# nomadkaraoke/python-audio-separator

Hardware: AMD Instinct MI355X
Metric: audio-sec separated / wall-sec (RTF), UVR-MDX-NET 44.1kHz stereo, 1/2/4/8 GPU (higher is better)
Workload: dtype f32 (I/O and accumulators; matrix products on the 16-bit pipe from block-scaled two-part fp16 operands, 22-bit products -- see arithmetic; fp32-exact setting timed in arithmetic_ab)

## Files before the change

python-audio-separator_amd/csrc/asx.hip:

```cpp
#include <hip/hip_runtime.h>

#include <algorithm>
#include <atomic>
#include <cmath>
#include <cstdarg>
#include <cstdio>
#include <cstdlib>
#include <cstring>
#include <functional>
#include <map>
#include <string>
#include <mutex>
#include <vector>

#include "../../include/asx.h"
#include "knobs.h"

static void grant_lds(const void *kernel, int bytes) {
  static std::mutex mu;
  static std::map<const void *, int> granted;
  std::lock_guard<std::mutex> lock(mu);
  int &g = granted[kernel];
  if (bytes > g) {
    (void)hipFuncSetAttribute(kernel, hipFuncAttributeMaxDynamicSharedMemorySize, bytes);
// ... 38 lines not shown
  const char *refusal = nullptr;
  int shipped = 0;
} kOptions[] = {
    {"winograd", &asx_engine::winograd, &EngineKnobs::winograd, opt_nonneg,
     "asx_set_option: winograd = %d names a superseded kernel generation that only an experimental build carries "
     "(python build.py --experimental); this library has 0 (direct kernel) and 3 (the default)", 3},
    {"winograd_stationary", &asx_engine::winos, &EngineKnobs::winos, opt_nonneg,
     "asx_set_option: the weight-stationary Winograd kernel (measured slower) is in experimental builds only (python build.py --experimental)"},
    {"winograd_bf16x6", &asx_engine::wino6, &EngineKnobs::wino6, opt_nonneg},
    {"gemm_bf16x6", &asx_engine::gemm_bf16x6, &EngineKnobs::gemm_bf16x6, opt_onoff},
    {"gemm_f16x3", &asx_engine::gemm_f16x3, &EngineKnobs::gemm_f16x3, opt_onoff},
    {"conv_direct_f16x3", &asx_engine::conv3h, &EngineKnobs::conv3h, opt_nonneg},
    {"conv_fuse_input", &asx_engine::conv_fuse_input, &EngineKnobs::conv_fuse_input, opt_onoff},
    {"conv_down_bf16x6", &asx_engine::down6, &EngineKnobs::down6, opt_onoff},
    {"conv_up_bf16x6", &asx_engine::up6, &EngineKnobs::up6, opt_onoff},
    {"gemm_pair_images", &asx_engine::pair_images, &EngineKnobs::pair_images, opt_onoff,
     "asx_set_option: gemm_pair_images = 1 needs an experimental build (python build.py --experimental): the pair-image reader measured no "
     "faster in the nets and is not in the default library"},
};

static const EngineOption *find_option(const char *fn, const char *key) {
  for (const EngineOption &o : kOptions)
    if (!strcmp(key, o.key)) return &o;
  set_err("%s: unknown option '%s'", fn, key);
  return nullptr;
}

extern "C" {

int asx_abi_version(void) { return ASX_ABI_VERSION; }
// ... 128 lines not shown
static void vr_destroy(VrNet *n);
static void ens_destroy(EnsCtx *c);
static void free_conv(ConvLayer &L) {
  L.w.release();
  L.b.release();
  L.wu.release();
  L.wu2.release();
  L.wu3.release();
  L.wus.release();
  L.wu6.release();
  L.wu6h.release();
  L.w3h.release();
  L.w1f.release();
  L.wd6.release();
  L.wup6.release();
  L.gn_w.release();
  L.gn_b.release();
}
static void free_tdf(TdfLayer &L) {
  L.w.release();
  L.bias.release();
  L.scale.release();
  L.shift.release();
  L.gn_w.release();
  L.gn_b.release();
}
static void free_block(Block &b) {
  for (auto &c : b.tfc) free_conv(c);
  free_tdf(b.tdf0);
  free_tdf(b.tdf1);
// ... 912 lines not shown
    kind = CK_DOWN;
    to = t / 2;
    fo = f / 2;
  } else if (!strcmp(op, "conv1x1")) kind = CK_1X1;
  else if (!strcmp(op, "up")) {
    kind = CK_UP;
    to = 2 * t;
    fo = 2 * f;
    REQUIRE(aux_host, "asx_op_conv(up): skip tensor required");
  } else {
    set_err("asx_op_conv: unknown op '%s'", op);
    return ASX_ERR_INVALID;
  }
  ConvLayer L;
  DevBuf dx, dy, dskip;
  BufGuard g{{&dx, &dy, &dskip, &L.w, &L.b, &L.wu, &L.wu2, &L.wu3, &L.wus, &L.wu6, &L.wu6h, &L.w3h, &L.wd6, &L.wup6}};
  CHK(conv_setup(L, kind, cin, cout, relu ? 1 : 0));
  CHK(conv_pack(L, w_host, b_host, e->winograd));
  CHK(to_dev(dx, x_host, (size_t)B * cin * t * f));
  const size_t ny = (size_t)B * cout * to * fo;
  CHK(dy.ensure(ny * 4));
  HIPCHK(hipMemset(dy.p, 0xff, ny * 4));
  if (kind == CK_UP) CHK(to_dev(dskip, aux_host, ny));
  CHK(conv_launch(e, L, dx.f(), dskip.f(), dy.f(), B, t, f, nullptr));
  CHK(to_host(y_host, dy, ny));
  return ASX_OK;
}

int asx_op_tdf(asx_engine *e, const float *x_host, int32_t B, int32_t c, int32_t t, int32_t k, const float *w_host,
               const float *bias_host, int32_t n, const float *scale_host, const float *shift_host,
               const float *res_host, float *y_host) {
// ... 934 lines not shown
int asx_counter(const asx_engine *e, const char *name, int64_t *out) {
  REQUIRE(e && name && out, "asx_counter: null argument");
  const std::string nm(name);
  if (nm == "tdf3_launches") *out = (int64_t)g_tdf3_launches.load();
  else if (nm == "tdf3h_launches") *out = (int64_t)g_tdf3h_launches.load();
  else if (nm == "attn6_launches") *out = (int64_t)g_attn6_launches.load();
  else if (nm == "attn6h_launches") *out = (int64_t)g_attn6h_launches.load();
  else if (nm == "tdf3_gather_launches") *out = (int64_t)g_tdf3_gather_launches.load();
  else if (nm == "wino6_launches") *out = (int64_t)g_wino6_launches.load();
  else if (nm == "wino6h_launches") *out = (int64_t)g_wino6h_launches.load();
  else if (nm == "conv3h_launches") *out = (int64_t)g_conv3h_launches.load();
  else if (nm == "conv3h_fin_launches") *out = (int64_t)g_conv3h_fin_launches.load();
  else if (nm == "tdf3_pair_image_launches") *out = (int64_t)g_tdf3ps_launches.load();
  else if (nm == "down6_launches") *out = (int64_t)g_down6_launches.load();
  else if (nm == "up6_launches") *out = (int64_t)g_up6_launches.load();
  else if (nm == "hd_rounds") *out = (int64_t)g_hd_rounds.load();
  else {
    set_err("asx_counter: unknown counter '%s'", name);
    return ASX_ERR_INVALID;
  }
  return ASX_OK;
}

int asx_debug_trace(uint64_t *host, int64_t n_u64) {
  REQUIRE(host && n_u64 > 0 && n_u64 <= 4096 * 8, "asx_debug_trace: bad argument");
  HIPCHK(hipDeviceSynchronize());
  HIPCHK(hipMemcpyFromSymbol(host, HIP_SYMBOL(asx_dbg_trace), (size_t)n_u64 * 8));
  return ASX_OK;
}

// ... 199 lines not shown
```

python-audio-separator_amd/csrc/engine_core.h:

```cpp
#pragma once

static thread_local char g_err[512] = "";
static void set_err(const char *fmt, ...) {
  va_list ap;
  va_start(ap, fmt);
  vsnprintf(g_err, sizeof(g_err), fmt, ap);
  va_end(ap);
}
#define HIPCHK(x)                                                                       \
  do {                                                                                  \
    hipError_t e_ = (x);                                                                \
    if (e_ != hipSuccess) {                                                             \
      set_err("%s:%d %s -> %s", __FILE__, __LINE__, #x, hipGetErrorString(e_));         \
      return ASX_ERR_HIP;                                                               \
    }                                                                                   \
  } while (0)
#define CHK(x)                    \
  do {                            \
    int r_ = (x);                 \
    if (r_ != ASX_OK) return r_;  \
  } while (0)
#define REQUIRE(cond, ...)        \
  do {                            \
    if (!(cond)) {                \
// ... 68 lines not shown
  DevBuf wu2;
  DevBuf wu3;
  int wu_cg = 0, wu_nci = 0, wu3_nci = 0;
  DevBuf wus;
  int wus_ks = 0;
  DevBuf gn_w, gn_b;
  DevBuf wu6;
  int wu6_nci = 0;
  DevBuf wu6h;
  DevBuf w3h;
  DevBuf w1f;
  DevBuf wd6;
  int wd6_cg = 0, wd6_nst = 0, wd6_nrep = 3;
  DevBuf wup6;
  int wup6_cg = 0, wup6_nst = 0;
};

struct TdfLayer {
  int n = 0, k = 0, c = 0;
  bool has_bias = false;
  DevBuf w, bias, scale, shift;
  DevBuf gn_w, gn_b;
};

struct Block {
  std::vector<ConvLayer> tfc;
  TdfLayer tdf0, tdf1;
  int c = 0, t = 0, f = 0;
};

// ... 64 lines not shown
  DevBuf d_div;
  DivKey div_key;
  DevBuf sinc_tab;
  hipEvent_t div_ev = nullptr;
  hipStream_t div_stream = nullptr;
  std::vector<DevBuf> skip;
  int winograd = 3;
  int winos = 0;
  int gemm_bf16x6 = 1;
  int gemm_f16x3 = 1;
  int wino6 = 144;
  int conv3h = 144;
  int conv_fuse_input = 1;
  int down6 = 1;
  int up6 = 1;
  int pair_images = 0;
  std::vector<W3Entry> w3;
  std::mutex w3_mu;
  bool prof = false;
  int prof_nprod = 0;
  std::vector<ProfRec> recs;
};

static int pick_batch(const asx_engine *e) { return e->cfg.max_batch > 0 ? e->cfg.max_batch : 64; }

static int even_batches(int nk, int maxB) {
  const int nbatch = (nk + maxB - 1) / maxB;
  return (nk + nbatch - 1) / nbatch;
}

// ... 74 lines not shown
```

python-audio-separator_amd/csrc/engine_mdx.h:

```cpp
#pragma once

template <class CFG>
static void launch_conv_t(const ConvArgs &a, int nblk, hipStream_t s) {
  grant_lds(&conv_mfma_kernel<CFG>, CFG::LDS_BYTES);
  hipLaunchKernelGGL(conv_mfma_kernel<CFG>, dim3(nblk), dim3(256), CFG::LDS_BYTES, s, a);
}

static int conv_tile_h(int kind) { return kind == CK_UP ? 4 : 8; }

static int pick_nrep_conv(int cout) {
  const int ct = (cout + 15) / 16;
  int best = 1, best_pad = 1 << 30;
  for (int n = 3; n >= 1; --n) {
    const int pad = ((ct + n - 1) / n) * n - ct;
    if (pad < best_pad) {
      best_pad = pad;
      best = n;
    }
  }
  return best;
}
static int pick_nrep_up(int cout) {
  const int ct = (cout + 15) / 16;
  if (knobs().up_nrep == 4 && (4 * ct) % 4 == 0) return 4;
// ... 150 lines not shown
  }
  if (L.kind == CK_1X1 && L.cin == 4 && L.cout == Conv3hCfg::C) {
    std::vector<float> w1((size_t)Conv3hCfg::C * 5, 0.f);
    memcpy(w1.data(), w, (size_t)Conv3hCfg::C * 4 * 4);
    if (b) memcpy(w1.data() + Conv3hCfg::C * 4, b, (size_t)Conv3hCfg::C * 4);
    CHK(L.w1f.ensure(w1.size() * 4));
    HIPCHK(hipMemcpy(L.w1f.p, w1.data(), w1.size() * 4, hipMemcpyHostToDevice));
  }
  if (L.kind == CK_DOWN) {
    std::vector<uint32_t> w6;
    L.wd6_nrep = (knobs().down6_wide && L.cout % 96 == 0) ? 6 : 3;
    if (L.wd6_nrep == 6) down6_pack<6>(w, L.cout, L.cin, w6, &L.wd6_cg, &L.wd6_nst);
    else down6_pack<3>(w, L.cout, L.cin, w6, &L.wd6_cg, &L.wd6_nst);
    CHK(L.wd6.ensure(w6.size() * 4));
    HIPCHK(hipMemcpy(L.wd6.p, w6.data(), w6.size() * 4, hipMemcpyHostToDevice));
  }
  if (L.kind == CK_UP) {
    std::vector<uint32_t> w6;
    if (L.nrep == 6) up6_pack<6>(w, L.cout, L.cin, w6, &L.wup6_cg, &L.wup6_nst);
    else if (L.nrep == 4) up6_pack<4>(w, L.cout, L.cin, w6, &L.wup6_cg, &L.wup6_nst);
    else up6_pack<2>(w, L.cout, L.cin, w6, &L.wup6_cg, &L.wup6_nst);
    CHK(L.wup6.ensure(w6.size() * 4));
    HIPCHK(hipMemcpy(L.wup6.p, w6.data(), w6.size() * 4, hipMemcpyHostToDevice));
  }
  const int nb = (L.kind == CK_UP) ? CT * 16 : std::max(L.cg * NW, ((L.cout + 47) / 48) * 48);
  std::vector<float> bp(nb, 0.f);
  for (int i = 0; i < L.cout; ++i) bp[i] = b ? b[i] : 0.f;
  CHK(L.w.ensure(wp.size() * 4));
  CHK(L.b.ensure(bp.size() * 4));
  HIPCHK(hipMemcpy(L.w.p, wp.data(), wp.size() * 4, hipMemcpyHostToDevice));
  HIPCHK(hipMemcpy(L.b.p, bp.data(), bp.size() * 4, hipMemcpyHostToDevice));
  return ASX_OK;
}

template <class CFG>
static void launch_conv_dma_t(const ConvArgs &a, int nblk, hipStream_t s) {
  grant_lds(&conv_dma_kernel<CFG>, CFG::LDS_BYTES);
  hipLaunchKernelGGL(conv_dma_kernel<CFG>, dim3(nblk), dim3(256), CFG::LDS_BYTES, s, a);
}

static std::atomic<long long> g_wino6_launches{0};
static std::atomic<long long> g_wino6h_launches{0};
static std::atomic<long long> g_conv3h_launches{0};
static std::atomic<long long> g_conv3h_fin_launches{0};
static std::atomic<long long> g_down6_launches{0};
static std::atomic<long long> g_up6_launches{0};

struct ConvView {
  int64_t x_bstride = 0;
  int64_t y_bstride = 0;
  const float *res = nullptr;
  int64_t aux_bstride = 0;
  int act = -1;
  float alpha = 1.f;
  const ConvLayer *fin = nullptr;
  const float *fin_x = nullptr;
};

static bool conv3h_takes(const asx_engine *e, const ConvLayer &L, bool dma, const float *res, int act, int T, int F, int64_t y_bstride, const float *y) {
#ifdef ASX_EXPERIMENTAL_KERNELS
  if (e->winos == 1 && L.wus.p != nullptr) return false;
// ... 227 lines not shown
    wa.wp = L.wu.f();
    wa.CG = L.wu_cg;
    wa.NCI = L.wu_nci;
    wa.tilesT = (a.To + WinoCfg::TH - 1) / WinoCfg::TH;
    wa.tilesF = (a.Fo + WinoCfg::TW - 1) / WinoCfg::TW;
    const int nb = wa.CG * wa.tilesT * wa.tilesF * B;
    grant_lds(&conv_wino_kernel, WinoCfg::LDS_BYTES);
    return timed(e, cls, flops, bytes, s, [&]() {
      hipLaunchKernelGGL(conv_wino_kernel, dim3(nb), dim3(256), WinoCfg::LDS_BYTES, s, wa);
    });
  }
#endif
  if (L.kind == CK_DOWN && e->gemm_bf16x6 > 0 && e->down6 > 0 && L.wd6.p != nullptr && dma && (a.Fo & 3) == 0 && (reinterpret_cast<uintptr_t>(y) & 15) == 0 &&
      a.y_bstride % 4 == 0 && (v.res == nullptr || ((reinterpret_cast<uintptr_t>(v.res) & 15) == 0 && a.aux_bstride % 4 == 0))) {
    ConvArgs da = a;
    da.wp = reinterpret_cast<const float *>(L.wd6.p);
    da.CG = L.wd6_cg;
    da.NCI = L.wd6_nst;
    da.tilesT = (a.To + Down6Cfg::TH - 1) / Down6Cfg::TH;
    da.tilesF = (a.Fo + Down6Cfg::TW - 1) / Down6Cfg::TW;
    const int nb6 = da.CG * da.tilesT * da.tilesF * B;
    grant_lds(&conv_down6_kernel<3>, Down6CfgT<3>::LDS_BYTES);
    grant_lds(&conv_down6_kernel<6>, Down6CfgT<6>::LDS_BYTES);
    g_down6_launches.fetch_add(1);
    return timed(e, cls, flops, bytes, s, [&]() {
      e->prof_nprod = 6;
      if (L.wd6_nrep == 6) hipLaunchKernelGGL(conv_down6_kernel<6>, dim3(nb6), dim3(256), Down6CfgT<6>::LDS_BYTES, s, da);
      else hipLaunchKernelGGL(conv_down6_kernel<3>, dim3(nb6), dim3(256), Down6CfgT<3>::LDS_BYTES, s, da);
    });
  }
  if (L.kind == CK_UP && e->gemm_bf16x6 > 0 && e->up6 > 0 && L.wup6.p != nullptr && dma && (reinterpret_cast<uintptr_t>(y) & 15) == 0 && a.y_bstride % 4 == 0 &&
      (skip == nullptr || ((reinterpret_cast<uintptr_t>(skip) & 15) == 0 && a.aux_bstride % 4 == 0))) {
    ConvArgs ua = a;
    ua.wp = reinterpret_cast<const float *>(L.wup6.p);
    ua.CG = L.wup6_cg;
    ua.NCI = L.wup6_nst;
    ua.tilesT = (T + 1) / 2;
    ua.tilesF = (F + 63) / 64;
    const int nbu = ua.CG * ua.tilesT * ua.tilesF * B;
    grant_lds(&conv_up6_kernel<6>, Up6CfgT<6>::LDS_BYTES);
    grant_lds(&conv_up6_kernel<4>, Up6CfgT<4>::LDS_BYTES);
    grant_lds(&conv_up6_kernel<2>, Up6CfgT<2>::LDS_BYTES);
    g_up6_launches.fetch_add(1);
    return timed(e, cls, flops, bytes, s, [&]() {
      e->prof_nprod = 6;
      if (L.nrep == 6) hipLaunchKernelGGL(conv_up6_kernel<6>, dim3(nbu), dim3(256), Up6CfgT<6>::LDS_BYTES, s, ua);
      else if (L.nrep == 4) hipLaunchKernelGGL(conv_up6_kernel<4>, dim3(nbu), dim3(256), Up6CfgT<4>::LDS_BYTES, s, ua);
      else hipLaunchKernelGGL(conv_up6_kernel<2>, dim3(nbu), dim3(256), Up6CfgT<2>::LDS_BYTES, s, ua);
    });
  }
#define ASX_CONV_CASE(KH, KW, S, PAD, NR, KC, RPW, EPI)                                      \
  do {                                                                                       \
    if (dma) launch_conv_dma_t<ConvDmaCfg<KH, KW, S, PAD, NR, KC, RPW, EPI>>(d, nblk, s);    \
    else launch_conv_t<ConvCfg<KH, KW, S, PAD, NR, KC, RPW, EPI>>(a, nblk, s);               \
  } while (0)
  CHK(timed(e, cls, flops, bytes, s, [&]() {
    switch (L.kind) {
      case CK_3X3:
        if (L.nrep == 3 && L.kc == 4) ASX_CONV_CASE(3, 3, 1, 1, 3, 4, 2, EPI_BIAS_ACT);
        else if (L.nrep == 3) ASX_CONV_CASE(3, 3, 1, 1, 3, 8, 2, EPI_BIAS_ACT);
        else if (L.nrep == 2 && L.kc == 4) ASX_CONV_CASE(3, 3, 1, 1, 2, 4, 2, EPI_BIAS_ACT);
// ... 690 lines not shown
```

python-audio-separator_amd/csrc/kernels_updown6.h:

```cpp
#pragma once
#include "kernels_gemm3.h"

namespace asx {

template <int NREP_, int TH_ = 2>
struct Down6CfgT {
  static constexpr int TH = TH_, TW = 64, KC = 8, NREP = NREP_, NW = 16 * NREP_;
  static constexpr int IH = 2 * TH, IWA = 2 * TW;
  static constexpr int PLANE = IH * IWA;
  static constexpr int NJ = PLANE / 256;
  static constexpr int PAIRS = TH / 2;
  static constexpr int PS = PLANE + 16;
  static constexpr int XBYTES = KC * PS * 4;
  static constexpr int WSTAGE_U32 = 3 * NREP * 64 * 4;
  static constexpr int BUF = XBYTES + WSTAGE_U32 * 4;
  static constexpr int LDS_BYTES = BUF;
};
typedef Down6CfgT<3> Down6Cfg;

static inline uint16_t down6_bf16_rne(float v) {
  uint32_t u;
  memcpy(&u, &v, 4);
  if ((u & 0x7f800000u) == 0x7f800000u) return (uint16_t)((u >> 16) | ((u & 0xffffu) ? 0x40u : 0u));
  u += 0x7fffu + ((u >> 16) & 1u);
  return (uint16_t)(u >> 16);
}
static inline float down6_bf16_f(uint16_t h) {
  const uint32_t u = (uint32_t)h << 16;
  float f;
  memcpy(&f, &u, 4);
  return f;
}

template <int NREP>
static inline void down6_pack(const float *w, int cout, int cin, std::vector<uint32_t> &img, int *cg_out, int *nst_out) {
  using Down6Cfg = Down6CfgT<NREP>;
  const int cg = (cout + Down6Cfg::NW - 1) / Down6Cfg::NW, nst = (cin + Down6Cfg::KC - 1) / Down6Cfg::KC;
  img.assign((size_t)cg * nst * Down6Cfg::WSTAGE_U32, 0u);
  uint16_t *o = reinterpret_cast<uint16_t *>(img.data());
  for (int g = 0; g < cg; ++g)
    for (int st = 0; st < nst; ++st)
      for (int n = 0; n < Down6Cfg::NREP; ++n)
        for (int lane = 0; lane < 64; ++lane) {
          const int co = g * Down6Cfg::NW + n * 16 + (lane & 15), lk = lane >> 4;
          for (int e = 0; e < 2; ++e)
            for (int tap = 0; tap < 4; ++tap) {
              const int c = st * Down6Cfg::KC + 2 * lk + e;
              const float v = (co < cout && c < cin) ? w[((size_t)co * cin + c) * 4 + tap] : 0.f;
              const uint16_t h = down6_bf16_rne(v);
              const float r1 = v - down6_bf16_f(h);
              const uint16_t m = down6_bf16_rne(r1);
              const uint16_t l = down6_bf16_rne(r1 - down6_bf16_f(m));
              const uint16_t parts[3] = {h, m, l};
              for (int p = 0; p < 3; ++p)
                o[((((size_t)(g * nst + st) * 3 + p) * Down6Cfg::NREP + n) * 64 + lane) * 8 + e * 4 + tap] = parts[p];
            }
        }
  if (cg_out) *cg_out = cg;
  if (nst_out) *nst_out = nst;
}

template <int NREP>
__device__ __forceinline__ void updown6_products(const u32x4 *w_s, int lane, const bf16x8 (&xh)[2], const bf16x8 (&xm)[2], const bf16x8 (&xl)[2],
// ... 15 lines not shown
    for (int n = 0; n < NREP; ++n) acc[m][n] = ASX_MFMA_BF16(xh[m], bw[n], acc[m][n]);
  }
#pragma unroll
  for (int n = 0; n < NREP; ++n) bw[n] = __builtin_bit_cast(bf16x8, w_s[n * 64 + lane]);
#pragma unroll
  for (int m = 0; m < 2; ++m) {
#pragma unroll
    for (int n = 0; n < NREP; ++n) acc[m][n] = ASX_MFMA_BF16(xl[m], bw[n], acc[m][n]);
#pragma unroll
    for (int n = 0; n < NREP; ++n) acc[m][n] = ASX_MFMA_BF16(xm[m], bw[n], acc[m][n]);
#pragma unroll
    for (int n = 0; n < NREP; ++n) acc[m][n] = ASX_MFMA_BF16(xh[m], bw[n], acc[m][n]);
  }
}

template <int NREP, int TH = 2>
__global__ __launch_bounds__(256, TH == 2 ? 4 : 3) void conv_down6_kernel(ConvArgs a) {
  using C = Down6CfgT<NREP, TH>;
  extern __shared__ float lds_f[];
  char *lds = reinterpret_cast<char *>(lds_f);
  const int tid = threadIdx.x, lane = tid & 63;
  const int wave = __builtin_amdgcn_readfirstlane(tid >> 6);
  const int li = lane & 15, lk = lane >> 4;

  int lid = xcd_remap(blockIdx.x, gridDim.x);
  const int cg = lid % a.CG;
  lid /= a.CG;
  const int tf = lid % a.tilesF;
  lid /= a.tilesF;
  const int tt = lid % a.tilesT;
  const int b = lid / a.tilesT;
  const int to0 = tt * C::TH, fo0 = tf * C::TW;
  const int ti0 = 2 * to0, fa0 = 2 * fo0;
// ... 17 lines not shown
    uint32_t *w_s = reinterpret_cast<uint32_t *>(lds + buf * C::BUF + C::XBYTES);
#pragma unroll
    for (int p = 0; p < 2; ++p) {
      const int pl = wave + 4 * p;
      const int c = st * C::KC + pl;
      const float *xc = xb + (int64_t)c * plane_sz;
      const bool cok = c < a.Cin;
#pragma unroll
      for (int j = 0; j < C::NJ; ++j) {
        const float *src = (cok && sp_ok[j]) ? xc + sp_off[j] : a.zeros;
        ASX_GLDS16(src, in_s + pl * C::PS + j * 256);
      }
    }
    const uint32_t *ws = wg + (int64_t)st * C::WSTAGE_U32;
#pragma unroll
    for (int i = 0; i < (3 * C::NREP + 3) / 4; ++i) {
      const int q = wave + 4 * i;
      if (q < 3 * C::NREP) ASX_GLDS16(ws + q * 256 + lane * 4, w_s + q * 256);
    }
  };

  f32x4 acc[C::PAIRS][2][C::NREP];
#pragma unroll
  for (int pi = 0; pi < C::PAIRS; ++pi)
#pragma unroll
    for (int m = 0; m < 2; ++m)
#pragma unroll
      for (int n = 0; n < C::NREP; ++n) acc[pi][m][n] = (f32x4){0.f, 0.f, 0.f, 0.f};

  const int row = TH == 2 ? (wave >> 1) : wave;
  for (int st = 0; st < a.NCI; ++st) {
    if (st > 0) __syncthreads();
    issue(st, 0);
    asm volatile("s_waitcnt vmcnt(0)" ::: "memory");
    __syncthreads();
    const float *in_s = reinterpret_cast<const float *>(lds);
    const u32x4 *w_s = reinterpret_cast<const u32x4 *>(lds + C::XBYTES);
#pragma unroll
    for (int pi = 0; pi < C::PAIRS; ++pi) {
      const int col0 = TH == 2 ? (wave & 1) * 2 : 2 * pi;
      bf16x8 xh[2], xm[2], xl[2];
#pragma unroll
      for (int m = 0; m < 2; ++m) {
        const float *p0 = in_s + (2 * lk) * C::PS + (2 * row) * C::IWA + 2 * ((col0 + m) * 16 + li);
        const f32x2 c0d0 = *reinterpret_cast<const f32x2 *>(p0);
        const f32x2 c0d1 = *reinterpret_cast<const f32x2 *>(p0 + C::IWA);
        const f32x2 c1d0 = *reinterpret_cast<const f32x2 *>(p0 + C::PS);
        const f32x2 c1d1 = *reinterpret_cast<const f32x2 *>(p0 + C::PS + C::IWA);
        unsigned hh[4], mm[4], ll[4];
        split3_pair(c0d0.x, c0d0.y, hh[0], mm[0], ll[0]);
        split3_pair(c0d1.x, c0d1.y, hh[1], mm[1], ll[1]);
        split3_pair(c1d0.x, c1d0.y, hh[2], mm[2], ll[2]);
        split3_pair(c1d1.x, c1d1.y, hh[3], mm[3], ll[3]);
        xh[m] = __builtin_bit_cast(bf16x8, (u32x4){hh[0], hh[1], hh[2], hh[3]});
        xm[m] = __builtin_bit_cast(bf16x8, (u32x4){mm[0], mm[1], mm[2], mm[3]});
        xl[m] = __builtin_bit_cast(bf16x8, (u32x4){ll[0], ll[1], ll[2], ll[3]});
      }
      updown6_products<C::NREP>(w_s, lane, xh, xm, xl, acc[pi]);
    }
  }

  const int t = to0 + row;
  if (t >= a.To) return;
  float *yb = a.y + (int64_t)b * a.y_bstride;
  const float *rb = a.res ? a.res + (int64_t)b * a.aux_bstride : nullptr;
#pragma unroll
  for (int n = 0; n < C::NREP; ++n) {
    const int co = cg * C::NW + n * 16 + li;
    if (co >= a.Cout) continue;
    const float bv = a.bias[co];
#pragma unroll
    for (int pi = 0; pi < C::PAIRS; ++pi)
#pragma unroll
      for (int m = 0; m < 2; ++m) {
        const int col0 = TH == 2 ? (wave & 1) * 2 : 2 * pi;
        const int f = fo0 + (col0 + m) * 16 + lk * 4;
        const int64_t off = ((int64_t)co * a.To + t) * a.Fo + f;
        const f32x4 v = acc[pi][m][n];
        if ((a.Fo & 3) == 0 && f + 4 <= a.Fo) {
          f32x4 o;
          o.x = act_fn(v.x + bv, a.act);
          o.y = act_fn(v.y + bv, a.act);
          o.z = act_fn(v.z + bv, a.act);
          o.w = act_fn(v.w + bv, a.act);
          if (rb != nullptr) o += *reinterpret_cast<const f32x4 *>(rb + off);
          *reinterpret_cast<f32x4 *>(yb + off) = o;
        } else {
          const float ov[4] = {v.x, v.y, v.z, v.w};
#pragma unroll
          for (int r = 0; r < 4; ++r)
            if (f + r < a.Fo) yb[off + r] = act_fn(ov[r] + bv, a.act) + (rb != nullptr ? rb[off + r] : 0.f);
        }
      }
  }
}

template <int NREP_>
struct Up6CfgT {
  static constexpr int TH = 2, TW = 64, KC = 32, NREP = NREP_;
  static constexpr int PAIR = 2 * TH * TW + 16;
  static constexpr int XBYTES = (KC / 2) * PAIR * 4;
  static constexpr int WSTAGE_U32 = 3 * NREP * 64 * 4;
  static constexpr int BUF = XBYTES + WSTAGE_U32 * 4;
  static constexpr int NBUF = 1;
  static constexpr int LDS_BYTES = NBUF * BUF;
};

template <int NREP>
static inline void up6_pack(const float *w, int cout, int cin, std::vector<uint32_t> &img, int *cg_out, int *nst_out) {
  using C = Up6CfgT<NREP>;
  const int CT = (cout + 15) / 16, vt = 4 * CT;
  const int cg = (vt + NREP - 1) / NREP, nst = (cin + C::KC - 1) / C::KC;
  img.assign((size_t)cg * nst * C::WSTAGE_U32, 0u);
  uint16_t *o = reinterpret_cast<uint16_t *>(img.data());
  for (int g = 0; g < cg; ++g)
    for (int st = 0; st < nst; ++st)
      for (int n = 0; n < NREP; ++n) {
        const int nt = g * NREP + n, pair = nt / 2, dx = nt & 1, dy = pair / CT, ct = pair % CT;
        for (int lane = 0; lane < 64; ++lane) {
          const int co = ct * 16 + (lane & 15), lk = lane >> 4;
          for (int kk = 0; kk < 8; ++kk) {
            const int c = st * C::KC + 2 * (lk + 4 * (kk >> 1)) + (kk & 1);
            const float v = (dy < 2 && co < cout && c < cin) ? w[(((size_t)c * cout + co) * 2 + dy) * 2 + dx] : 0.f;
            const uint16_t h = down6_bf16_rne(v);
            const float r1 = v - down6_bf16_f(h);
            const uint16_t m = down6_bf16_rne(r1);
            const uint16_t l = down6_bf16_rne(r1 - down6_bf16_f(m));
            const uint16_t parts[3] = {h, m, l};
            for (int p = 0; p < 3; ++p) o[((((size_t)(g * nst + st) * 3 + p) * NREP + n) * 64 + lane) * 8 + kk] = parts[p];
          }
        }
      }
  if (cg_out) *cg_out = cg;
  if (nst_out) *nst_out = nst;
}

template <int NREP>
__global__ __launch_bounds__(256, 4) void conv_up6_kernel(ConvArgs a) {
  using C = Up6CfgT<NREP>;
  static_assert(NREP % 2 == 0, "the dx tiles of a pair stay together");
  extern __shared__ float lds_f[];
  char *lds = reinterpret_cast<char *>(lds_f);
  const int tid = threadIdx.x, lane = tid & 63;
  const int wave = __builtin_amdgcn_readfirstlane(tid >> 6);
  const int li = lane & 15, lk = lane >> 4;

  int lid = xcd_remap(blockIdx.x, gridDim.x);
  const int cg = lid % a.CG;
  lid /= a.CG;
  const int tf = lid % a.tilesF;
  lid /= a.tilesF;
  const int tt = lid % a.tilesT;
  const int b = lid / a.tilesT;
  const int to0 = tt * C::TH, fo0 = tf * C::TW;
// ... 5 lines not shown
  const int slot = lane & 31, srow = slot >> 4, sc4 = slot & 15;
  const bool sp_ok = (to0 + srow) < a.T && (fo0 + sc4 * 4) < a.F;
  const int sp_off = (to0 + srow) * a.F + fo0 + sc4 * 4;
  auto issue = [&](int st, int buf) {
    float *in_s = reinterpret_cast<float *>(lds + buf * C::BUF);
    uint32_t *w_s = reinterpret_cast<uint32_t *>(lds + buf * C::BUF + C::XBYTES);
#pragma unroll
    for (int i = 0; i < 4; ++i) {
      const int pr = wave + 4 * i;
      const int c = st * C::KC + 2 * pr + (lane >> 5);
      const float *src = (c < a.Cin && sp_ok) ? xb + (int64_t)c * plane_sz + sp_off : a.zeros;
      ASX_GLDS16(src, in_s + pr * C::PAIR);
    }
    const uint32_t *ws = wg + (int64_t)st * C::WSTAGE_U32;
#pragma unroll
    for (int i = 0; i < (3 * NREP + 3) / 4; ++i) {
      const int q = wave + 4 * i;
      if (q < 3 * NREP) ASX_GLDS16(ws + q * 256 + lane * 4, w_s + q * 256);
    }
  };

  f32x4 acc[2][NREP];
#pragma unroll
  for (int m = 0; m < 2; ++m)
#pragma unroll
    for (int n = 0; n < NREP; ++n) acc[m][n] = (f32x4){0.f, 0.f, 0.f, 0.f};

  const int row = wave >> 1, col0 = (wave & 1) * 2;
  for (int st = 0; st < a.NCI; ++st) {
    if (st > 0) __syncthreads();
    issue(st, 0);
    asm volatile("s_waitcnt vmcnt(0)" ::: "memory");
    __syncthreads();
    const float *in_s = reinterpret_cast<const float *>(lds);
    const u32x4 *w_s = reinterpret_cast<const u32x4 *>(lds + C::XBYTES);
    bf16x8 xh[2], xm[2], xl[2];
#pragma unroll
    for (int m = 0; m < 2; ++m) {
      const float *p0 = in_s + lk * C::PAIR + row * C::TW + (col0 + m) * 16 + li;
      unsigned hh[4], mm[4], ll[4];
#pragma unroll
      for (int jj = 0; jj < 4; ++jj) {
        const float v0 = p0[jj * 4 * C::PAIR], v1 = p0[jj * 4 * C::PAIR + C::TH * C::TW];
        split3_pair(v0, v1, hh[jj], mm[jj], ll[jj]);
      }
      xh[m] = __builtin_bit_cast(bf16x8, (u32x4){hh[0], hh[1], hh[2], hh[3]});
      xm[m] = __builtin_bit_cast(bf16x8, (u32x4){mm[0], mm[1], mm[2], mm[3]});
      xl[m] = __builtin_bit_cast(bf16x8, (u32x4){ll[0], ll[1], ll[2], ll[3]});
    }
    updown6_products<NREP>(w_s, lane, xh, xm, xl, acc);
// ... 1 lines not shown

  const int t = to0 + row;
  if (t >= a.T) return;
  const int CT = (a.Cout + 15) / 16;
  const int To2 = a.T * 2, Fo2 = a.F * 2;
  float *yb = a.y + (int64_t)b * a.y_bstride;
  const float *sb = a.skip ? a.skip + (int64_t)b * a.aux_bstride : nullptr;
#pragma unroll
  for (int np = 0; np < NREP / 2; ++np) {
    const int pair = (cg * NREP) / 2 + np;
    const int dy = pair / CT, ct = pair - dy * CT;
    if (dy >= 2) continue;
    const int co = ct * 16 + li;
    if (co >= a.Cout) continue;
    const float bv = a.bias[co];
    f32x4 s0[2], s1[2];
#pragma unroll
    for (int m = 0; m < 2; ++m) {
      const int f = fo0 + (col0 + m) * 16 + lk * 4;
      const int64_t off = ((int64_t)co * To2 + (2 * t + dy)) * Fo2 + 2 * f;
      const bool in = sb != nullptr && f + 4 <= a.F;
      s0[m] = in ? *reinterpret_cast<const f32x4 *>(sb + off) : (f32x4){1.f, 1.f, 1.f, 1.f};
      s1[m] = in ? *reinterpret_cast<const f32x4 *>(sb + off + 4) : (f32x4){1.f, 1.f, 1.f, 1.f};
    }
#pragma unroll
    for (int m = 0; m < 2; ++m) {
      const int f = fo0 + (col0 + m) * 16 + lk * 4;
      if (f >= a.F) continue;
      const int64_t off = ((int64_t)co * To2 + (2 * t + dy)) * Fo2 + 2 * f;
      const f32x4 v0 = acc[m][2 * np], v1 = acc[m][2 * np + 1];
      if (f + 4 <= a.F) {
        f32x4 r0, r1;
        r0.x = act_fn(v0.x + bv, a.act);
        r0.y = act_fn(v1.x + bv, a.act);
        r0.z = act_fn(v0.y + bv, a.act);
        r0.w = act_fn(v1.y + bv, a.act);
        r1.x = act_fn(v0.z + bv, a.act);
        r1.y = act_fn(v1.z + bv, a.act);
        r1.z = act_fn(v0.w + bv, a.act);
        r1.w = act_fn(v1.w + bv, a.act);
        r0 *= s0[m];
        r1 *= s1[m];
        *reinterpret_cast<f32x4 *>(yb + off) = r0;
        *reinterpret_cast<f32x4 *>(yb + off + 4) = r1;
      } else {
// ... 11 lines not shown
```

python-audio-separator_amd/csrc/knobs.h:

```cpp
#pragma once

#include <algorithm>
#include <climits>
#include <cstdint>
#include <cstdlib>

#ifndef ASX_TDF2_DEFAULT
#define ASX_TDF2_DEFAULT 1
#endif

constexpr int HD_MAX_GROUPS = 6;

namespace knob {
inline bool set(const char *name) { return getenv(name) != nullptr; }
inline int num(const char *name, int def) { return set(name) ? atoi(getenv(name)) : def; }
inline int64_t num64(const char *name, int64_t def) { return set(name) ? atoll(getenv(name)) : def; }
inline double real(const char *name, double def) { return set(name) ? atof(getenv(name)) : def; }
inline bool on_unless_0(const char *name) { return !(set(name) && atoi(getenv(name)) == 0); }
inline bool off_unless_nonzero(const char *name) { return set(name) && atoi(getenv(name)) != 0; }
inline int clamped(const char *name, int def, int lo, int hi = INT_MAX) { return set(name) ? std::max(lo, std::min(hi, atoi(getenv(name)))) : def; }
}

struct Knobs {
  int poison = knob::num("ASX_POISON", -1);
// ... 68 lines not shown
  int winograd = knob::clamped("ASX_WINOGRAD", 3, 0);
  int winos = knob::clamped("ASX_WINOS", 0, 0);
  int pair_images = knob::num("ASX_PAIR_IMAGES", 0);
#else
  int winograd = knob::num("ASX_WINOGRAD", 3) <= 0 ? 0 : 3;
  int winos = 0;
  int pair_images = 0;
#endif
  int gemm_bf16x6 = knob::num("ASX_GEMM_BF16X6", 1);
  int gemm_f16x3 = knob::num("ASX_GEMM_F16X3", 1);
  int wino6 = knob::clamped("ASX_WINO6", 144, 0);
  int conv3h = knob::clamped("ASX_CONV3H", 144, 0);
  int conv_fuse_input = 1;
  int down6 = knob::num("ASX_DOWN6", 1);
  int up6 = knob::num("ASX_UP6", 1);
  bool fft3 = knob::on_unless_0("ASX_FFT3");
  bool fft3p = knob::on_unless_0("ASX_FFT3P");
};
```

Before: 1578.

## Add block-scaled two-part fp16 variants of the down/up convolution kernels

Adds f16x3 variants of the strided down-conv and transposed up-conv kernels. Weights are packed as scaled fp16 hi/lo pairs with a per-output-channel exponent, and activations are split on the fly with a running wave-wide exponent. This needs three MFMA products per tile instead of six bf16 products, and the weight tile staged in LDS shrinks from three parts to two. The variants are on by default whenever gemm_f16x3 is enabled. The cost is more in-kernel work for the activation split and rescaling, plus a different rounding profile that depends on the dynamic exponent tracking.

```diff
diff --git a/python-audio-separator_amd/csrc/asx.hip b/python-audio-separator_amd/csrc/asx.hip
--- a/python-audio-separator_amd/csrc/asx.hip
+++ b/python-audio-separator_amd/csrc/asx.hip
@@ -76,6 +76,7 @@
     {"conv_fuse_input", &asx_engine::conv_fuse_input, &EngineKnobs::conv_fuse_input, opt_onoff},
     {"conv_down_bf16x6", &asx_engine::down6, &EngineKnobs::down6, opt_onoff},
     {"conv_up_bf16x6", &asx_engine::up6, &EngineKnobs::up6, opt_onoff},
+    {"conv_updown_f16x3", &asx_engine::updown_f16x3, &EngineKnobs::updown_f16x3, opt_onoff},
     {"gemm_pair_images", &asx_engine::pair_images, &EngineKnobs::pair_images, opt_onoff,
      "asx_set_option: gemm_pair_images = 1 needs an experimental build (python build.py --experimental): the pair-image reader measured no "
      "faster in the nets and is not in the default library"},
@@ -234,6 +235,8 @@
   L.w1f.release();
   L.wd6.release();
   L.wup6.release();
+  L.wd6h.release();
+  L.wup6h.release();
   L.gn_w.release();
   L.gn_b.release();
 }
@@ -1176,7 +1179,7 @@
   }
   ConvLayer L;
   DevBuf dx, dy, dskip;
-  BufGuard g{{&dx, &dy, &dskip, &L.w, &L.b, &L.wu, &L.wu2, &L.wu3, &L.wus, &L.wu6, &L.wu6h, &L.w3h, &L.wd6, &L.wup6}};
+  BufGuard g{{&dx, &dy, &dskip, &L.w, &L.b, &L.wu, &L.wu2, &L.wu3, &L.wus, &L.wu6, &L.wu6h, &L.w3h, &L.wd6, &L.wup6, &L.wd6h, &L.wup6h}};
   CHK(conv_setup(L, kind, cin, cout, relu ? 1 : 0));
   CHK(conv_pack(L, w_host, b_host, e->winograd));
   CHK(to_dev(dx, x_host, (size_t)B * cin * t * f));
@@ -2141,6 +2144,8 @@
   else if (nm == "tdf3_pair_image_launches") *out = (int64_t)g_tdf3ps_launches.load();
   else if (nm == "down6_launches") *out = (int64_t)g_down6_launches.load();
   else if (nm == "up6_launches") *out = (int64_t)g_up6_launches.load();
+  else if (nm == "down6h_launches") *out = (int64_t)g_down6h_launches.load();
+  else if (nm == "up6h_launches") *out = (int64_t)g_up6h_launches.load();
   else if (nm == "hd_rounds") *out = (int64_t)g_hd_rounds.load();
   else {
     set_err("asx_counter: unknown counter '%s'", name);
diff --git a/python-audio-separator_amd/csrc/engine_core.h b/python-audio-separator_amd/csrc/engine_core.h
--- a/python-audio-separator_amd/csrc/engine_core.h
+++ b/python-audio-separator_amd/csrc/engine_core.h
@@ -106,6 +106,7 @@
   int wd6_cg = 0, wd6_nst = 0, wd6_nrep = 3;
   DevBuf wup6;
   int wup6_cg = 0, wup6_nst = 0;
+  DevBuf wd6h, wup6h;
 };
 
 struct TdfLayer {
@@ -200,6 +201,7 @@
   int conv_fuse_input = 1;
   int down6 = 1;
   int up6 = 1;
+  int updown_f16x3 = 1;
   int pair_images = 0;
   std::vector<W3Entry> w3;
   std::mutex w3_mu;
diff --git a/python-audio-separator_amd/csrc/engine_mdx.h b/python-audio-separator_amd/csrc/engine_mdx.h
--- a/python-audio-separator_amd/csrc/engine_mdx.h
+++ b/python-audio-separator_amd/csrc/engine_mdx.h
@@ -188,6 +188,10 @@
     else down6_pack<3>(w, L.cout, L.cin, w6, &L.wd6_cg, &L.wd6_nst);
     CHK(L.wd6.ensure(w6.size() * 4));
     HIPCHK(hipMemcpy(L.wd6.p, w6.data(), w6.size() * 4, hipMemcpyHostToDevice));
+    if (L.wd6_nrep == 6) down6_pack<6, true>(w, L.cout, L.cin, w6, nullptr, nullptr);
+    else down6_pack<3, true>(w, L.cout, L.cin, w6, nullptr, nullptr);
+    CHK(L.wd6h.ensure(w6.size() * 4));
+    HIPCHK(hipMemcpy(L.wd6h.p, w6.data(), w6.size() * 4, hipMemcpyHostToDevice));
   }
   if (L.kind == CK_UP) {
     std::vector<uint32_t> w6;
@@ -196,6 +200,11 @@
     else up6_pack<2>(w, L.cout, L.cin, w6, &L.wup6_cg, &L.wup6_nst);
     CHK(L.wup6.ensure(w6.size() * 4));
     HIPCHK(hipMemcpy(L.wup6.p, w6.data(), w6.size() * 4, hipMemcpyHostToDevice));
+    if (L.nrep == 6) up6_pack<6, true>(w, L.cout, L.cin, w6, nullptr, nullptr);
+    else if (L.nrep == 4) up6_pack<4, true>(w, L.cout, L.cin, w6, nullptr, nullptr);
+    else up6_pack<2, true>(w, L.cout, L.cin, w6, nullptr, nullptr);
+    CHK(L.wup6h.ensure(w6.size() * 4));
+    HIPCHK(hipMemcpy(L.wup6h.p, w6.data(), w6.size() * 4, hipMemcpyHostToDevice));
   }
   const int nb = (L.kind == CK_UP) ? CT * 16 : std::max(L.cg * NW, ((L.cout + 47) / 48) * 48);
   std::vector<float> bp(nb, 0.f);
@@ -219,6 +228,9 @@
 static std::atomic<long long> g_conv3h_fin_launches{0};
 static std::atomic<long long> g_down6_launches{0};
 static std::atomic<long long> g_up6_launches{0};
+static std::atomic<long long> g_down6h_launches{0};
+static std::atomic<long long> g_up6h_launches{0};
+constexpr int UPDOWN_H_MIN_CIN = 0;
 
 struct ConvView {
   int64_t x_bstride = 0;
@@ -476,7 +488,8 @@
   if (L.kind == CK_DOWN && e->gemm_bf16x6 > 0 && e->down6 > 0 && L.wd6.p != nullptr && dma && (a.Fo & 3) == 0 && (reinterpret_cast<uintptr_t>(y) & 15) == 0 &&
       a.y_bstride % 4 == 0 && (v.res == nullptr || ((reinterpret_cast<uintptr_t>(v.res) & 15) == 0 && a.aux_bstride % 4 == 0))) {
     ConvArgs da = a;
-    da.wp = reinterpret_cast<const float *>(L.wd6.p);
+    const bool h3 = e->gemm_f16x3 > 0 && e->updown_f16x3 > 0 && L.wd6h.p != nullptr && L.cin >= UPDOWN_H_MIN_CIN;
+    da.wp = reinterpret_cast<const float *>(h3 ? L.wd6h.p : L.wd6.p);
     da.CG = L.wd6_cg;
     da.NCI = L.wd6_nst;
     da.tilesT = (a.To + Down6Cfg::TH - 1) / Down6Cfg::TH;
@@ -484,17 +497,23 @@
     const int nb6 = da.CG * da.tilesT * da.tilesF * B;
     grant_lds(&conv_down6_kernel<3>, Down6CfgT<3>::LDS_BYTES);
     grant_lds(&conv_down6_kernel<6>, Down6CfgT<6>::LDS_BYTES);
+    grant_lds(&conv_down6_kernel<3, 2, true>, Down6CfgT<3, 2, true>::LDS_BYTES);
+    grant_lds(&conv_down6_kernel<6, 2, true>, Down6CfgT<6, 2, true>::LDS_BYTES);
     g_down6_launches.fetch_add(1);
+    if (h3) g_down6h_launches.fetch_add(1);
     return timed(e, cls, flops, bytes, s, [&]() {
-      e->prof_nprod = 6;
-      if (L.wd6_nrep == 6) hipLaunchKernelGGL(conv_down6_kernel<6>, dim3(nb6), dim3(256), Down6CfgT<6>::LDS_BYTES, s, da);
+      e->prof_nprod = h3 ? 3 : 6;
+      if (h3 && L.wd6_nrep == 6) hipLaunchKernelGGL((conv_down6_kernel<6, 2, true>), dim3(nb6), dim3(256), (Down6CfgT<6, 2, true>::LDS_BYTES), s, da);
+      else if (h3) hipLaunchKernelGGL((conv_down6_kernel<3, 2, true>), dim3(nb6), dim3(256), (Down6CfgT<3, 2, true>::LDS_BYTES), s, da);
+      else if (L.wd6_nrep == 6) hipLaunchKernelGGL(conv_down6_kernel<6>, dim3(nb6), dim3(256), Down6CfgT<6>::LDS_BYTES, s, da);
       else hipLaunchKernelGGL(conv_down6_kernel<3>, dim3(nb6), dim3(256), Down6CfgT<3>::LDS_BYTES, s, da);
     });
   }
   if (L.kind == CK_UP && e->gemm_bf16x6 > 0 && e->up6 > 0 && L.wup6.p != nullptr && dma && (reinterpret_cast<uintptr_t>(y) & 15) == 0 && a.y_bstride % 4 == 0 &&
       (skip == nullptr || ((reinterpret_cast<uintptr_t>(skip) & 15) == 0 && a.aux_bstride % 4 == 0))) {
     ConvArgs ua = a;
-    ua.wp = reinterpret_cast<const float *>(L.wup6.p);
+    const bool h3 = e->gemm_f16x3 > 0 && e->updown_f16x3 > 0 && L.wup6h.p != nullptr && L.cin >= UPDOWN_H_MIN_CIN;
+    ua.wp = reinterpret_cast<const float *>(h3 ? L.wup6h.p : L.wup6.p);
     ua.CG = L.wup6_cg;
     ua.NCI = L.wup6_nst;
     ua.tilesT = (T + 1) / 2;
@@ -503,10 +522,17 @@
     grant_lds(&conv_up6_kernel<6>, Up6CfgT<6>::LDS_BYTES);
     grant_lds(&conv_up6_kernel<4>, Up6CfgT<4>::LDS_BYTES);
     grant_lds(&conv_up6_kernel<2>, Up6CfgT<2>::LDS_BYTES);
+    grant_lds(&conv_up6_kernel<6, true>, Up6CfgHT<6, true>::LDS_BYTES);
+    grant_lds(&conv_up6_kernel<4, true>, Up6CfgHT<4, true>::LDS_BYTES);
+    grant_lds(&conv_up6_kernel<2, true>, Up6CfgHT<2, true>::LDS_BYTES);
     g_up6_launches.fetch_add(1);
+    if (h3) g_up6h_launches.fetch_add(1);
     return timed(e, cls, flops, bytes, s, [&]() {
-      e->prof_nprod = 6;
-      if (L.nrep == 6) hipLaunchKernelGGL(conv_up6_kernel<6>, dim3(nbu), dim3(256), Up6CfgT<6>::LDS_BYTES, s, ua);
+      e->prof_nprod = h3 ? 3 : 6;
+      if (h3 && L.nrep == 6) hipLaunchKernelGGL((conv_up6_kernel<6, true>), dim3(nbu), dim3(256), (Up6CfgHT<6, true>::LDS_BYTES), s, ua);
+      else if (h3 && L.nrep == 4) hipLaunchKernelGGL((conv_up6_kernel<4, true>), dim3(nbu), dim3(256), (Up6CfgHT<4, true>::LDS_BYTES), s, ua);
+      else if (h3) hipLaunchKernelGGL((conv_up6_kernel<2, true>), dim3(nbu), dim3(256), (Up6CfgHT<2, true>::LDS_BYTES), s, ua);
+      else if (L.nrep == 6) hipLaunchKernelGGL(conv_up6_kernel<6>, dim3(nbu), dim3(256), Up6CfgT<6>::LDS_BYTES, s, ua);
       else if (L.nrep == 4) hipLaunchKernelGGL(conv_up6_kernel<4>, dim3(nbu), dim3(256), Up6CfgT<4>::LDS_BYTES, s, ua);
       else hipLaunchKernelGGL(conv_up6_kernel<2>, dim3(nbu), dim3(256), Up6CfgT<2>::LDS_BYTES, s, ua);
     });
diff --git a/python-audio-separator_amd/csrc/kernels_updown6.h b/python-audio-separator_amd/csrc/kernels_updown6.h
--- a/python-audio-separator_amd/csrc/kernels_updown6.h
+++ b/python-audio-separator_amd/csrc/kernels_updown6.h
@@ -1,10 +1,12 @@
 #pragma once
 #include "kernels_gemm3.h"
+#include "kernels_conv3h.h"
 
 namespace asx {
 
-template <int NREP_, int TH_ = 2>
+template <int NREP_, int TH_ = 2, bool H_ = false>
 struct Down6CfgT {
+  static constexpr int WPARTS = H_ ? 2 : 3;
   static constexpr int TH = TH_, TW = 64, KC = 8, NREP = NREP_, NW = 16 * NREP_;
   static constexpr int IH = 2 * TH, IWA = 2 * TW;
   static constexpr int PLANE = IH * IWA;
@@ -12,7 +14,7 @@
   static constexpr int PAIRS = TH / 2;
   static constexpr int PS = PLANE + 16;
   static constexpr int XBYTES = KC * PS * 4;
-  static constexpr int WSTAGE_U32 = 3 * NREP * 64 * 4;
+  static constexpr int WSTAGE_U32 = WPARTS * NREP * 64 * 4;
   static constexpr int BUF = XBYTES + WSTAGE_U32 * 4;
   static constexpr int LDS_BYTES = BUF;
 };
@@ -32,12 +34,53 @@
   return f;
 }
 
-template <int NREP>
+static inline uint16_t down6_f16_rne(float v) {
+  uint32_t u;
+  memcpy(&u, &v, 4);
+  const uint16_t sign = (uint16_t)((u >> 16) & 0x8000u);
+  const float a = std::fabs(v);
+  if (!(a == a)) return (uint16_t)(sign | 0x7e00u);
+  if (a < 6.103515625e-5f) return (uint16_t)(sign | (uint16_t)std::nearbyint(std::ldexp((double)a, 24)));
+  if (a >= 65520.f) return (uint16_t)(sign | 0x7c00u);
+  int e;
+  const double f = std::frexp((double)a, &e);
+  int m = (int)std::nearbyint(std::ldexp(f, 11));
+  if (m == 2048) {
+    m = 1024;
+    ++e;
+  }
+  return (uint16_t)(sign | ((e - 1 + 15) << 10) | (m - 1024));
+}
+static inline float down6_f16_f(uint16_t h) {
+  const int ex = (h >> 10) & 31, m = h & 0x3ff;
+  float f;
+  if (ex == 0) f = std::ldexp((float)m, -24);
+  else if (ex == 31) f = m ? NAN : INFINITY;
+  else f = std::ldexp((float)(1024 + m), ex - 25);
+  return (h & 0x8000u) ? -f : f;
+}
+static inline int down6_f16_exp(float mx) {
+  if (!(mx > 0.f) || std::isinf(mx)) return 0;
+  int fe;
+  (void)std::frexp(mx, &fe);
+  return 15 - fe;
+}
+
+template <int NREP, bool H = false>
 static inline void down6_pack(const float *w, int cout, int cin, std::vector<uint32_t> &img, int *cg_out, int *nst_out) {
-  using Down6Cfg = Down6CfgT<NREP>;
+  using Down6Cfg = Down6CfgT<NREP, 2, H>;
   const int cg = (cout + Down6Cfg::NW - 1) / Down6Cfg::NW, nst = (cin + Down6Cfg::KC - 1) / Down6Cfg::KC;
-  img.assign((size_t)cg * nst * Down6Cfg::WSTAGE_U32, 0u);
+  img.assign((size_t)cg * nst * Down6Cfg::WSTAGE_U32 + (H ? (size_t)cg * Down6Cfg::NW : 0), 0u);
   uint16_t *o = reinterpret_cast<uint16_t *>(img.data());
+  std::vector<int> ex(H ? (size_t)cg * Down6Cfg::NW : 0, 0);
+  if (H) {
+    for (int co = 0; co < cout; ++co) {
+      float mx = 0.f;
+      for (int i = 0; i < cin * 4; ++i) mx = std::max(mx, std::fabs(w[(size_t)co * cin * 4 + i]));
+      ex[co] = down6_f16_exp(mx);
+      img[(size_t)cg * nst * Down6Cfg::WSTAGE_U32 + co] = (uint32_t)ex[co];
+    }
+  }
   for (int g = 0; g < cg; ++g)
     for (int st = 0; st < nst; ++st)
       for (int n = 0; n < Down6Cfg::NREP; ++n)
@@ -47,6 +90,13 @@
             for (int tap = 0; tap < 4; ++tap) {
               const int c = st * Down6Cfg::KC + 2 * lk + e;
               const float v = (co < cout && c < cin) ? w[((size_t)co * cin + c) * 4 + tap] : 0.f;
+              if (H) {
+                const float vs = std::ldexp(v, ex[co]);
+                const uint16_t hh = down6_f16_rne(vs), lh = down6_f16_rne(vs - down6_f16_f(hh));
+                o[((((size_t)(g * nst + st) * 2 + 0) * Down6Cfg::NREP + n) * 64 + lane) * 8 + e * 4 + tap] = hh;
+                o[((((size_t)(g * nst + st) * 2 + 1) * Down6Cfg::NREP + n) * 64 + lane) * 8 + e * 4 + tap] = lh;
+                continue;
+              }
               const uint16_t h = down6_bf16_rne(v);
               const float r1 = v - down6_bf16_f(h);
               const uint16_t m = down6_bf16_rne(r1);
@@ -92,9 +142,52 @@
   }
 }
 
-template <int NREP, int TH = 2>
+template <int NREP>
+__device__ __forceinline__ void updown6_products(const u32x4 *w_s, int lane, const f16x8 (&xh)[2], const f16x8 (&xl)[2], f32x4 (&acc)[2][NREP]) {
+  f16x8 bw[NREP];
+#pragma unroll
+  for (int n = 0; n < NREP; ++n) bw[n] = __builtin_bit_cast(f16x8, w_s[(NREP + n) * 64 + lane]);
+#pragma unroll
+  for (int m = 0; m < 2; ++m)
+#pragma unroll
+    for (int n = 0; n < NREP; ++n) acc[m][n] = ASX_MFMA_F16(xh[m], bw[n], acc[m][n]);
+#pragma unroll
+  for (int n = 0; n < NREP; ++n) bw[n] = __builtin_bit_cast(f16x8, w_s[n * 64 + lane]);
+#pragma unroll
+  for (int m = 0; m < 2; ++m) {
+#pragma unroll
+    for (int n = 0; n < NREP; ++n) acc[m][n] = ASX_MFMA_F16(xl[m], bw[n], acc[m][n]);
+#pragma unroll
+    for (int n = 0; n < NREP; ++n) acc[m][n] = ASX_MFMA_F16(xh[m], bw[n], acc[m][n]);
+  }
+}
+
+template <int NREP>
+__device__ __forceinline__ void updown6_split_h(const float (&v)[8], int &em, int &em_lo, f32x4 (&acc)[NREP], f16x8 &xh, f16x8 &xl) {
+  float mx = fmaxf(fmaxf(fmaxf(fabsf(v[0]), fabsf(v[1])), fmaxf(fabsf(v[2]), fabsf(v[3]))), fmaxf(fmaxf(fabsf(v[4]), fabsf(v[5])), fmaxf(fabsf(v[6]), fabsf(v[7]))));
+  mx = wave_max64(mx);
+  const int need = min(__builtin_amdgcn_readfirstlane(f16_scale_exp(mx)), 100);
+  int e_new = em;
+  if (need < em) e_new = need - 2;
+  else if (need > em + F16X3_RISE && mx > 0.f) e_new = min(need - 2, em_lo + F16X3_RISE_CAP);
+  em_lo = min(em_lo, e_new);
+  if (e_new != em) {
+    const float fdev = __builtin_ldexpf(1.0f, e_new - em);
+#pragma unroll
+    for (int n = 0; n < NREP; ++n) acc[n] *= fdev;
+  }
+  em = e_new;
+  const float sc = __builtin_ldexpf(1.0f, e_new);
+  unsigned hh[4], ll[4];
+#pragma unroll
+  for (int i = 0; i < 4; ++i) conv3h_split_pair(v[2 * i], v[2 * i + 1], sc, hh[i], ll[i]);
+  xh = __builtin_bit_cast(f16x8, (u32x4){hh[0], hh[1], hh[2], hh[3]});
+  xl = __builtin_bit_cast(f16x8, (u32x4){ll[0], ll[1], ll[2], ll[3]});
+}
+
+template <int NREP, int TH = 2, bool H = false>
 __global__ __launch_bounds__(256, TH == 2 ? 4 : 3) void conv_down6_kernel(ConvArgs a) {
-  using C = Down6CfgT<NREP, TH>;
+  using C = Down6CfgT<NREP, TH, H>;
   extern __shared__ float lds_f[];
   char *lds = reinterpret_cast<char *>(lds_f);
   const int tid = threadIdx.x, lane = tid & 63;
@@ -142,12 +235,17 @@
     }
     const uint32_t *ws = wg + (int64_t)st * C::WSTAGE_U32;
 #pragma unroll
-    for (int i = 0; i < (3 * C::NREP + 3) / 4; ++i) {
+    for (int i = 0; i < (C::WPARTS * C::NREP + 3) / 4; ++i) {
       const int q = wave + 4 * i;
-      if (q < 3 * C::NREP) ASX_GLDS16(ws + q * 256 + lane * 4, w_s + q * 256);
+      if (q < C::WPARTS * C::NREP) ASX_GLDS16(ws + q * 256 + lane * 4, w_s + q * 256);
     }
   };
 
+  int em[C::PAIRS][2], em_lo[C::PAIRS][2];
+#pragma unroll
+  for (int pi = 0; pi < C::PAIRS; ++pi)
+#pragma unroll
+    for (int m = 0; m < 2; ++m) em[pi][m] = em_lo[pi][m] = 200;
   f32x4 acc[C::PAIRS][2][C::NREP];
 #pragma unroll
   for (int pi = 0; pi < C::PAIRS; ++pi)
@@ -167,6 +265,21 @@
 #pragma unroll
     for (int pi = 0; pi < C::PAIRS; ++pi) {
       const int col0 = TH == 2 ? (wave & 1) * 2 : 2 * pi;
+      if constexpr (H) {
+        f16x8 fh[2], fl[2];
+#pragma unroll
+        for (int m = 0; m < 2; ++m) {
+          const float *p0 = in_s + (2 * lk) * C::PS + (2 * row) * C::IWA + 2 * ((col0 + m) * 16 + li);
+          const f32x2 c0d0 = *reinterpret_cast<const f32x2 *>(p0);
+          const f32x2 c0d1 = *reinterpret_cast<const f32x2 *>(p0 + C::IWA);
+          const f32x2 c1d0 = *reinterpret_cast<const f32x2 *>(p0 + C::PS);
+          const f32x2 c1d1 = *reinterpret_cast<const f32x2 *>(p0 + C::PS + C::IWA);
+          const float v[8] = {c0d0.x, c0d0.y, c0d1.x, c0d1.y, c1d0.x, c1d0.y, c1d1.x, c1d1.y};
+          updown6_split_h<C::NREP>(v, em[pi][m], em_lo[pi][m], acc[pi][m], fh[m], fl[m]);
+        }
+        updown6_products<C::NREP>(w_s, lane, fh, fl, acc[pi]);
+        continue;
+      }
       bf16x8 xh[2], xm[2], xl[2];
 #pragma unroll
       for (int m = 0; m < 2; ++m) {
@@ -197,6 +310,8 @@
     const int co = cg * C::NW + n * 16 + li;
     if (co >= a.Cout) continue;
     const float bv = a.bias[co];
+    int ew = 0;
+    if constexpr (H) ew = reinterpret_cast<const int *>(a.wp)[(int64_t)a.CG * a.NCI * C::WSTAGE_U32 + cg * C::NW + n * 16 + li];
 #pragma unroll
     for (int pi = 0; pi < C::PAIRS; ++pi)
 #pragma unroll
@@ -204,7 +319,8 @@
         const int col0 = TH == 2 ? (wave & 1) * 2 : 2 * pi;
         const int f = fo0 + (col0 + m) * 16 + lk * 4;
         const int64_t off = ((int64_t)co * a.To + t) * a.Fo + f;
-        const f32x4 v = acc[pi][m][n];
+        f32x4 v = acc[pi][m][n];
+        if constexpr (H) ldexp4_inplace(v, -(em[pi][m] + ew));
         if ((a.Fo & 3) == 0 && f + 4 <= a.Fo) {
           f32x4 o;
           o.x = act_fn(v.x + bv, a.act);
@@ -234,13 +350,35 @@
   static constexpr int LDS_BYTES = NBUF * BUF;
 };
 
-template <int NREP>
+template <int NREP_, bool H_>
+struct Up6CfgHT : Up6CfgT<NREP_> {
+  static constexpr int WPARTS = H_ ? 2 : 3;
+  static constexpr int WSTAGE_U32 = WPARTS * NREP_ * 64 * 4;
+  static constexpr int BUF = Up6CfgT<NREP_>::XBYTES + WSTAGE_U32 * 4;
+  static constexpr int LDS_BYTES = BUF;
+};
+
+template <int NREP, bool H = false>
 static inline void up6_pack(const float *w, int cout, int cin, std::vector<uint32_t> &img, int *cg_out, int *nst_out) {
-  using C = Up6CfgT<NREP>;
+  using C = Up6CfgHT<NREP, H>;
   const int CT = (cout + 15) / 16, vt = 4 * CT;
   const int cg = (vt + NREP - 1) / NREP, nst = (cin + C::KC - 1) / C::KC;
-  img.assign((size_t)cg * nst * C::WSTAGE_U32, 0u);
+  img.assign((size_t)cg * nst * C::WSTAGE_U32 + (H ? (size_t)cg * NREP * 16 : 0), 0u);
   uint16_t *o = reinterpret_cast<uint16_t *>(img.data());
+  std::vector<int> ex(H ? (size_t)cg * NREP * 16 : 0, 0);
+  if (H) {
+    for (int nt = 0; nt < cg * NREP; ++nt) {
+      const int pair = nt / 2, dx = nt & 1, dy = pair / CT, ct = pair % CT;
+      for (int li = 0; li < 16; ++li) {
+        const int co = ct * 16 + li;
+        float mx = 0.f;
+        if (dy < 2 && co < cout)
+          for (int c = 0; c < cin; ++c) mx = std::max(mx, std::fabs(w[(((size_t)c * cout + co) * 2 + dy) * 2 + dx]));
+        ex[(size_t)nt * 16 + li] = down6_f16_exp(mx);
+        img[(size_t)cg * nst * C::WSTAGE_U32 + (size_t)nt * 16 + li] = (uint32_t)ex[(size_t)nt * 16 + li];
+      }
+    }
+  }
   for (int g = 0; g < cg; ++g)
     for (int st = 0; st < nst; ++st)
       for (int n = 0; n < NREP; ++n) {
@@ -250,6 +388,13 @@
           for (int kk = 0; kk < 8; ++kk) {
             const int c = st * C::KC + 2 * (lk + 4 * (kk >> 1)) + (kk & 1);
             const float v = (dy < 2 && co < cout && c < cin) ? w[(((size_t)c * cout + co) * 2 + dy) * 2 + dx] : 0.f;
+            if (H) {
+              const float vs = std::ldexp(v, ex[(size_t)nt * 16 + (lane & 15)]);
+              const uint16_t hh = down6_f16_rne(vs), lh = down6_f16_rne(vs - down6_f16_f(hh));
+              o[((((size_t)(g * nst + st) * 2 + 0) * NREP + n) * 64 + lane) * 8 + kk] = hh;
+              o[((((size_t)(g * nst + st) * 2 + 1) * NREP + n) * 64 + lane) * 8 + kk] = lh;
+              continue;
+            }
             const uint16_t h = down6_bf16_rne(v);
             const float r1 = v - down6_bf16_f(h);
             const uint16_t m = down6_bf16_rne(r1);
@@ -263,9 +408,9 @@
   if (nst_out) *nst_out = nst;
 }
 
-template <int NREP>
+template <int NREP, bool H = false>
 __global__ __launch_bounds__(256, 4) void conv_up6_kernel(ConvArgs a) {
-  using C = Up6CfgT<NREP>;
+  using C = Up6CfgHT<NREP, H>;
   static_assert(NREP % 2 == 0, "the dx tiles of a pair stay together");
   extern __shared__ float lds_f[];
   char *lds = reinterpret_cast<char *>(lds_f);
@@ -301,12 +446,13 @@
     }
     const uint32_t *ws = wg + (int64_t)st * C::WSTAGE_U32;
 #pragma unroll
-    for (int i = 0; i < (3 * NREP + 3) / 4; ++i) {
+    for (int i = 0; i < (C::WPARTS * NREP + 3) / 4; ++i) {
       const int q = wave + 4 * i;
-      if (q < 3 * NREP) ASX_GLDS16(ws + q * 256 + lane * 4, w_s + q * 256);
+      if (q < C::WPARTS * NREP) ASX_GLDS16(ws + q * 256 + lane * 4, w_s + q * 256);
     }
   };
 
+  int em[2] = {200, 200}, em_lo[2] = {200, 200};
   f32x4 acc[2][NREP];
 #pragma unroll
   for (int m = 0; m < 2; ++m)
@@ -321,6 +467,22 @@
     __syncthreads();
     const float *in_s = reinterpret_cast<const float *>(lds);
     const u32x4 *w_s = reinterpret_cast<const u32x4 *>(lds + C::XBYTES);
+    if constexpr (H) {
+      f16x8 fh[2], fl[2];
+#pragma unroll
+      for (int m = 0; m < 2; ++m) {
+        const float *p0 = in_s + lk * C::PAIR + row * C::TW + (col0 + m) * 16 + li;
+        float v[8];
+#pragma unroll
+        for (int jj = 0; jj < 4; ++jj) {
+          v[2 * jj] = p0[jj * 4 * C::PAIR];
+          v[2 * jj + 1] = p0[jj * 4 * C::PAIR + C::TH * C::TW];
+        }
+        updown6_split_h<NREP>(v, em[m], em_lo[m], acc[m], fh[m], fl[m]);
+      }
+      updown6_products<NREP>(w_s, lane, fh, fl, acc);
+      continue;
+    }
     bf16x8 xh[2], xm[2], xl[2];
 #pragma unroll
     for (int m = 0; m < 2; ++m) {
@@ -352,6 +514,12 @@
     const int co = ct * 16 + li;
     if (co >= a.Cout) continue;
     const float bv = a.bias[co];
+    int ew0 = 0, ew1 = 0;
+    if constexpr (H) {
+      const int *ewp = reinterpret_cast<const int *>(a.wp) + (int64_t)a.CG * a.NCI * C::WSTAGE_U32 + (cg * NREP + 2 * np) * 16 + li;
+      ew0 = ewp[0];
+      ew1 = ewp[16];
+    }
     f32x4 s0[2], s1[2];
 #pragma unroll
     for (int m = 0; m < 2; ++m) {
@@ -366,7 +534,11 @@
       const int f = fo0 + (col0 + m) * 16 + lk * 4;
       if (f >= a.F) continue;
       const int64_t off = ((int64_t)co * To2 + (2 * t + dy)) * Fo2 + 2 * f;
-      const f32x4 v0 = acc[m][2 * np], v1 = acc[m][2 * np + 1];
+      f32x4 v0 = acc[m][2 * np], v1 = acc[m][2 * np + 1];
+      if constexpr (H) {
+        ldexp4_inplace(v0, -(em[m] + ew0));
+        ldexp4_inplace(v1, -(em[m] + ew1));
+      }
       if (f + 4 <= a.F) {
         f32x4 r0, r1;
         r0.x = act_fn(v0.x + bv, a.act);
diff --git a/python-audio-separator_amd/csrc/knobs.h b/python-audio-separator_amd/csrc/knobs.h
--- a/python-audio-separator_amd/csrc/knobs.h
+++ b/python-audio-separator_amd/csrc/knobs.h
@@ -106,6 +106,7 @@
   int conv_fuse_input = 1;
   int down6 = knob::num("ASX_DOWN6", 1);
   int up6 = knob::num("ASX_UP6", 1);
+  int updown_f16x3 = 1;
   bool fft3 = knob::on_unless_0("ASX_FFT3");
   bool fft3p = knob::on_unless_0("ASX_FFT3P");
 };
```

Result: no change. 1591 (median of 6 runs) (+0.8%).
